# rotationalio/honu

Measured on AMD Instinct MI355X. Metric: GiB/s + records/s device-resident encode+decode, 1M Large(~300KB) object batch, higher is better.
Workload: dtype u8

## Files before the change

honu_amd/csrc/api.hip:

```cpp
#include <stdio.h>
#include <stdlib.h>
#include <string.h>

#include "kernels.h"

using namespace honu;

struct honu_ctx {
    int device;
    uint64_t max_n;
    LaunchGeom geom;
    void *ws;
    uint64_t *counts;
    uint64_t *offs;
    uint64_t *totals;
    DecodeScratch *scratch;
    uint32_t *reg_inline;
    EncAclPos *enc_acl;
    FusedState dec;
    uint64_t lb_bytes;
    ScanState scan;
    uint32_t spec_off;
    int speculate;
    hipStream_t aux;
// ... 24 lines not shown
    return HONU_E_HIP;
}
#define HIPCHK(x)                                  \
    do {                                           \
        hipError_t e_ = (x);                       \
        if (e_ != hipSuccess) return hip_fail(e_, #x); \
    } while (0)

static int32_t arg_fail(const char *what) {
    snprintf(g_last_error, sizeof g_last_error, "invalid argument: %s", what);
    return HONU_E_ARG;
}

static bool aligned(const void *p, uintptr_t a) { return ((uintptr_t)p & (a - 1)) == 0; }

#define FUSED_DECODE_MIN_RECORDS (48ull << 10)

static int fused_blocks(const LaunchGeom &g) {
    const int resident = 2 * g.num_cu;
    return g.lane_blocks > 0 && g.lane_blocks < resident ? g.lane_blocks : resident;
}

template <class T>
static uint64_t carve(T *&p, void *base, uint64_t at, uint64_t count) {
    p = (T *)((uintptr_t)base + at);
    return at + count * sizeof(T);
}

static uint64_t ctx_carve(honu_ctx *c, void *base) {
    const uint64_t n = c->max_n;
    const uint64_t tiles = (n + HONU_WAVE - 1) / HONU_WAVE;
    const uint64_t groups = (tiles / HONU_WAVE + 1) > LB_GROUPS ? tiles / HONU_WAVE + 1 : LB_GROUPS;
    uint64_t at = 0;
    at = carve(c->counts, base, at, 3 * n);
    at = carve(c->offs, base, at, 3 * n);
    at = carve(c->totals, base, at, 4);
    at = carve(c->scratch, base, at, n);
    at = carve(c->reg_inline, base, at, 8 * n);
    at = carve(c->enc_acl, base, at, n);
    at = carve(c->dec.lb, base, at, 1);
    at = carve(c->scan.lb, base, at, 1);
    at = carve(c->dec.status, base, at, 3 * tiles);
    at = carve(c->dec.gstatus, base, at, 3 * groups);
    c->dec.words = 3 * tiles + 3 * groups;
    c->scan.words = scan_status_words(n);
    at = carve(c->scan.status, base, at, c->scan.words);
    return carve(c->geom.copy_tickets, base, at, (uint64_t)COPY_TICKET_LINES * COPY_TICKET_STRIDE);
}

static bool stream_is_restricted(hipStream_t s, int num_cu) {
    int prio = 0;
    if (hipStreamGetPriority(s, &prio) == hipSuccess && prio != 0) return true;
    uint32_t mask[32] = {0};
    const uint32_t words = (uint32_t)((num_cu + 31) / 32);
    if (words > 32 || hipExtStreamGetCUMask(s, words, mask) != hipSuccess) return false;
    bool any = false, all = true;
    for (int i = 0; i < num_cu; i++) {
        const bool on = mask[i / 32] >> (i % 32) & 1u;
        any |= on;
        all &= on;
    }
    return any && !all;
}

static int env_int(const char *name, int dflt) {
#ifdef HONU_AB
    const char *v = getenv(name);
    return v && *v ? atoi(v) : dflt;
#else
    (void)name;
    return dflt;
#endif
}

extern "C" {

uint32_t honu_abi_version(void) { return HONU_ABI_VERSION; }
uint64_t honu_sizeof_meta(void) { return sizeof(honu_meta); }
uint64_t honu_sizeof_acl(void) { return sizeof(honu_acl); }
uint64_t honu_sizeof_collection(void) { return sizeof(honu_collection); }
uint64_t honu_sizeof_index(void) { return sizeof(honu_index); }
uint64_t honu_sizeof_record_info(void) { return sizeof(honu_record_info); }
uint64_t honu_sizeof_seek(void) { return sizeof(honu_seek); }
uint64_t honu_sizeof_list_row(void) { return sizeof(honu_list_row); }
uint64_t honu_sizeof_next(void) { return sizeof(honu_next); }
const char *honu_last_error(void) { return g_last_error; }

const char *honu_status_string(int32_t st) {
    switch (st) {
    case HONU_OK: return "ok";
    case HONU_ERR_BAD_VERSION: return "object is malformed: cannot decode specified version";
    case HONU_ERR_MALFORMED: return "object is malformed: cannot parse data or metadata";
    case HONU_ERR_EOF: return "EOF";
    case HONU_ERR_UNEXPECTED_EOF: return "unexpected EOF";
    case HONU_ERR_NO_LENGTH: return "field not written with length value";
    case HONU_ERR_PARSE_BOOLEAN: return "could not parse boolean value";
    case HONU_ERR_PARSE_VARINT: return "could not parse varint";
    case HONU_ERR_PANIC: return "input on which the Go reference panics";
    case HONU_ERR_CAPACITY: return "output capacity exceeded";
    case HONU_ERR_INPUT: return "input span or list outside its arena";
    case HONU_UNPARSED: return "metadata not decoded (headers only)";
    case HONU_E_ARG: return "invalid argument";
    case HONU_E_WORKSPACE: return "batch larger than the context's reserved records";
    case HONU_E_HIP: return "HIP runtime error";
    case HONU_E_NO_DEVICE: return "no gfx950 device";
    default: return "unknown status";
    }
}

honu_ctx *honu_ctx_create(int device, uint64_t max_records, int32_t *err) {
    int32_t dummy;
    if (!err) err = &dummy;
    *err = HONU_OK;
    int count = 0;
    if (hipGetDeviceCount(&count) != hipSuccess || device < 0 || device >= count) {
        snprintf(g_last_error, sizeof g_last_error, "no HIP device %d (count %d)", device, count);
        *err = HONU_E_NO_DEVICE;
        return nullptr;
    }
    hipDeviceProp_t prop;
    if (hipGetDeviceProperties(&prop, device) != hipSuccess ||
        strncmp(prop.gcnArchName, "gfx950", 6) != 0) {
        snprintf(g_last_error, sizeof g_last_error, "device %d is %s, this build targets gfx950",
                 device, prop.gcnArchName);
        *err = HONU_E_NO_DEVICE;
        return nullptr;
    }
    if (hipSetDevice(device) != hipSuccess) {
        *err = HONU_E_HIP;
        return nullptr;
    }
    honu_ctx *c = (honu_ctx *)calloc(1, sizeof(honu_ctx));
    if (!c) {
        *err = HONU_E_HIP;
        return nullptr;
    }
    auto fail = [&](int32_t e, const char *what) -> honu_ctx * {
        if (what) snprintf(g_last_error, sizeof g_last_error, "%s", what);
        if (c->ev_join) (void)hipEventDestroy(c->ev_join);
        if (c->ev_fork) (void)hipEventDestroy(c->ev_fork);
        if (c->aux) (void)hipStreamDestroy(c->aux);
        if (c->dec.spec_seen) (void)hipHostFree(c->dec.spec_seen);
        if (c->ws) (void)hipFree(c->ws);
        free(c);
        *err = e;
        return nullptr;
    };
    c->device = device;
    c->max_n = max_records ? max_records : 1;
    c->geom.num_cu = prop.multiProcessorCount;
    c->geom.per_record_blocks = env_int("HONU_RECORD_BLOCKS", prop.multiProcessorCount * 8);
    c->geom.lane_blocks = env_int("HONU_LANE_BLOCKS", 0);
    c->geom.copy_blocks = env_int("HONU_COPY_BLOCKS", prop.multiProcessorCount * 2);
    c->geom.record_variant = env_int("HONU_RECORD_VARIANT", 0);
    if (c->geom.record_variant != 5 && c->geom.record_variant != 6)
        c->geom.record_variant = 0;
    c->acl_inplace = env_int("HONU_ACL_INPLACE", 1) != 0;
    c->reg_inplace = env_int("HONU_REGIONS_INPLACE", 1) != 0;
    c->guard_blocks = env_int("HONU_GUARD_BLOCKS", 0);
    if (c->guard_blocks < 0) c->guard_blocks = 0;
    const uint64_t end = ctx_carve(c, nullptr), bytes = end + 256;
    if (hipMalloc(&c->ws, bytes) != hipSuccess) {
        c->ws = nullptr;
        char msg[96];
        snprintf(msg, sizeof msg, "hipMalloc(%llu) failed", (unsigned long long)bytes);
        return fail(HONU_E_HIP, msg);
    }
    if (hipHostMalloc((void **)&c->dec.spec_seen, 2 * sizeof(uint32_t),
                      hipHostMallocMapped | hipHostMallocCoherent) != hipSuccess) {
        c->dec.spec_seen = nullptr;
        return fail(HONU_E_HIP, "hipHostMalloc(spec_seen) failed");
    }
    c->dec.spec_seen[0] = 0;
    c->dec.spec_seen[1] = 0;
    c->speculate = SPECULATE_DEFAULT;
    c->enc_fork = env_int("HONU_ENCODE_FORK", 2);
    if (c->enc_fork < 0 || c->enc_fork > 2) c->enc_fork = 2;
    if (hipStreamCreateWithFlags(&c->aux, hipStreamNonBlocking) != hipSuccess) {
        c->aux = nullptr;
        return fail(HONU_E_HIP, "stream creation failed");
    }
    if (hipEventCreateWithFlags(&c->ev_fork, hipEventDisableTiming) != hipSuccess) {
        c->ev_fork = nullptr;
        return fail(HONU_E_HIP, "event creation failed");
    }
    if (hipEventCreateWithFlags(&c->ev_join, hipEventDisableTiming) != hipSuccess) {
        c->ev_join = nullptr;
        return fail(HONU_E_HIP, "event creation failed");
    }
    ctx_carve(c, c->ws);
    c->lb_bytes = (uint64_t)((uint8_t *)c->ws + end - (uint8_t *)c->dec.lb);
    c->geom.copy_steal = 1;
    c->scan.max_blocks = 4 * prop.multiProcessorCount;
    hipStream_t s = nullptr;
    bool ok = hipStreamCreateWithFlags(&s, hipStreamNonBlocking) == hipSuccess;
    ok = ok && hipMemsetAsync(c->dec.lb, 0, c->lb_bytes, s) == hipSuccess;
    ok = ok && hipStreamSynchronize(s) == hipSuccess;
    if (s) (void)hipStreamDestroy(s);
    if (!ok) return fail(HONU_E_HIP, "look-back state initialisation failed");
    return c;
}

int32_t honu_ctx_reset(honu_ctx *ctx, void *stream) {
    if (!ctx) return arg_fail("ctx");
    HIPCHK(hipSetDevice(ctx->device));
    HIPCHK(hipMemsetAsync(ctx->dec.lb, 0, ctx->lb_bytes, (hipStream_t)stream));
    HIPCHK(hipStreamSynchronize((hipStream_t)stream));
    return HONU_OK;
}

void honu_ctx_destroy(honu_ctx *ctx) {
    if (!ctx) return;
    (void)hipSetDevice(ctx->device);
    (void)hipStreamSynchronize(ctx->aux);
    (void)hipEventDestroy(ctx->ev_fork);
    (void)hipEventDestroy(ctx->ev_join);
    (void)hipStreamDestroy(ctx->aux);
    (void)hipFree(ctx->ws);
    (void)hipHostFree(ctx->dec.spec_seen);
    free(ctx);
}

uint64_t honu_ctx_max_records(const honu_ctx *ctx) { return ctx ? ctx->max_n : 0; }

int32_t honu_ctx_set_param(honu_ctx *ctx, const char *name, int64_t value) {
    if (!ctx || !name) return arg_fail("ctx/name");
    if (!strcmp(name, "copy_blocks") && value > 0) ctx->geom.copy_blocks = (int)value;
    else if (!strcmp(name, "record_blocks") && value > 0) ctx->geom.per_record_blocks = (int)value;
    else if (!strcmp(name, "lane_blocks") && value >= 0) ctx->geom.lane_blocks = (int)value;
    else if (!strcmp(name, "speculate") && value >= 0 && value <= 2) ctx->speculate = (int)value;
    else if (!strcmp(name, "encode_fork") && value >= 0 && value <= 2) ctx->enc_fork = (int)value;
    else if (!strcmp(name, "acl_inplace") && (value == 0 || value == 1)) ctx->acl_inplace = value != 0;
    else if (!strcmp(name, "regions_inplace") && (value == 0 || value == 1)) ctx->reg_inplace = value != 0;
    else if (!strcmp(name, "guard_blocks") && value >= 0 && value <= 65536) ctx->guard_blocks = (int)value;
    else if (!strcmp(name, "speculate_backoff") && value >= 0 && value <= (int64_t)SPEC_BACKOFF_CALLS) {
        __atomic_store_n(ctx->dec.spec_seen, 0u, __ATOMIC_RELAXED);
        ctx->spec_off = (uint32_t)value;
    }
    else if (!strcmp(name, "copy_steal") && (value == 0 || value == 1)) ctx->geom.copy_steal = (int)value;
    else if (!strcmp(name, "copy_variant") || !strcmp(name, "encode_variant") || !strcmp(name, "inline_recovery")) {
        if (value != 0) return arg_fail(name);
    }
    else if (!strcmp(name, "record_variant") &&
             (value == 0 || value == 5 || value == 6))
        ctx->geom.record_variant = (int)value;
    else if (!strcmp(name, "seek_variant") && value >= 0 && value <= 2) ctx->geom.seek_variant = (int)value;
    else return arg_fail(name);
    return HONU_OK;
}

int32_t honu_ctx_get_param(const honu_ctx *ctx, const char *name, int64_t *value) {
    if (!ctx || !name || !value) return arg_fail("ctx/name/value");
    if (!strcmp(name, "copy_blocks")) *value = ctx->geom.copy_blocks;
    else if (!strcmp(name, "record_blocks")) *value = ctx->geom.per_record_blocks;
    else if (!strcmp(name, "lane_blocks")) *value = ctx->geom.lane_blocks;
    else if (!strcmp(name, "speculate")) *value = ctx->speculate;
    else if (!strcmp(name, "encode_fork")) *value = ctx->enc_fork;
    else if (!strcmp(name, "acl_inplace")) *value = ctx->acl_inplace ? 1 : 0;
    else if (!strcmp(name, "regions_inplace")) *value = ctx->reg_inplace ? 1 : 0;
    else if (!strcmp(name, "guard_blocks")) *value = ctx->guard_blocks;
    else if (!strcmp(name, "recoveries"))
        *value = __atomic_load_n(ctx->dec.spec_seen + 1, __ATOMIC_RELAXED);
    else if (!strcmp(name, "speculate_backoff"))
        *value = __atomic_load_n(ctx->dec.spec_seen, __ATOMIC_RELAXED) ? SPEC_BACKOFF_CALLS : ctx->spec_off;
    else if (!strcmp(name, "copy_steal")) *value = ctx->geom.copy_steal;
    else if (!strcmp(name, "copy_variant") || !strcmp(name, "encode_variant") || !strcmp(name, "inline_recovery"))
        *value = 0;
    else if (!strcmp(name, "record_variant")) *value = ctx->geom.record_variant;
    else if (!strcmp(name, "walk_flag_checks")) *value = decode_walk_flag_checks();
    else if (!strcmp(name, "sort_tile")) *value = sort_tile();
    else if (!strcmp(name, "seek_variant")) *value = ctx->geom.seek_variant;
    else if (!strcmp(name, "seek_fence")) *value = seek_fence();
    else if (!strcmp(name, "seek_auto_probes")) *value = (int64_t)seek_auto_probes();
    else if (!strcmp(name, "seek_auto_keys")) *value = (int64_t)seek_auto_keys();
    else if (!strcmp(name, "merge_tile")) *value = merge_tile();
    else if (!strcmp(name, "delete_tile")) *value = delete_tile();
    else if (!strcmp(name, "list_tile")) *value = list_tile();
    else if (!strcmp(name, "list_stage")) *value = list_stage();
    else if (!strcmp(name, "filter_tile")) *value = filter_tile();
    else if (!strcmp(name, "compare_tile")) *value = compare_tile();
    else if (!strcmp(name, "compare_stage")) *value = compare_stage();
    else return arg_fail(name);
    return HONU_OK;
}

int32_t honu_encode_sizes(honu_ctx *ctx, const honu_meta *d_meta, uint64_t var_len,
                          const honu_acl *d_acl, uint64_t acl_len, const uint32_t *d_regions,
                          uint64_t regions_len, const uint64_t *d_payload_off, uint64_t n,
                          uint64_t *d_sizes, int32_t *d_status, void *stream) {
    if (!ctx) return arg_fail("ctx");
    if (n && (!d_meta || !d_payload_off || !d_sizes)) return arg_fail("null pointer");
    if (!aligned(d_meta, 16)) return arg_fail("rows must be 16-byte aligned");
    if (!aligned(d_acl, 4) || !aligned(d_regions, 4)) return arg_fail("tables must be 4-byte aligned");
    HIPCHK(hipSetDevice(ctx->device));
    HIPCHK(launch_encode_sizes_grp(d_meta, var_len, d_acl, acl_len, d_regions, regions_len,
                                   d_payload_off, n, d_sizes, d_status, ctx->geom.lane_blocks,
                                   (hipStream_t)stream));
    return HONU_OK;
}

int32_t honu_exclusive_scan(honu_ctx *ctx, const uint64_t *d_in, uint64_t n, uint64_t *d_out,
                            void *stream) {
    if (!ctx) return arg_fail("ctx");
    if (n > ctx->max_n) return HONU_E_WORKSPACE;
    HIPCHK(hipSetDevice(ctx->device));
    HIPCHK(launch_scan(d_in, n, 1, d_out, d_out + n, ctx->scan, (hipStream_t)stream));
    return HONU_OK;
}

static int32_t encode_records(honu_ctx *ctx, const honu_meta *d_meta, const uint8_t *d_var,
                              const honu_acl *d_acl, const uint32_t *d_regions, const uint8_t *units,
                              const uint64_t *d_payload_off, uint64_t n, uint8_t *d_out,
                              uint64_t out_cap, const uint64_t *d_out_off, int32_t *d_status,
                              void *stream) {
    if (!ctx) return arg_fail("ctx");
    if (n && (!d_meta || !d_payload_off || !d_out || !d_out_off || !d_status))
        return arg_fail("null pointer");
    if (!aligned(d_out, 16) || !aligned(d_meta, 16))
        return arg_fail("records arena and rows must be 16-byte aligned");
    if (!aligned(d_acl, 4) || !aligned(d_regions, 4)) return arg_fail("tables must be 4-byte aligned");
    HIPCHK(hipSetDevice(ctx->device));
    if (n > ctx->max_n) return HONU_E_WORKSPACE;
    ctx->enc_form = units ? 2 : 1;
    hipStream_t s = (hipStream_t)stream;
    const bool fork = ctx->enc_fork == 1 ||
                      (ctx->enc_fork == 2 && ctx->geom.lane_blocks > 0 && n &&
                       !stream_is_restricted(s, ctx->geom.num_cu));
    if (fork && n) {
        HIPCHK(hipEventRecord(ctx->ev_fork, s));
        HIPCHK(hipStreamWaitEvent(ctx->aux, ctx->ev_fork, 0));
        HIPCHK(launch_encode_acl_grp_self(d_meta, d_acl, d_payload_off, n, d_out, out_cap, d_out_off, d_status,
                                          ctx->geom.lane_blocks, ctx->aux));
        HIPCHK(hipEventRecord(ctx->ev_join, ctx->aux));
        HIPCHK(launch_encode_meta_lane(d_meta, d_var, d_acl, d_regions, d_payload_off, n, d_out,
                                       out_cap, d_out_off, d_status, ctx->enc_acl,
                                       ctx->geom.lane_blocks, ctx->geom.num_cu, units, s));
        HIPCHK(hipStreamWaitEvent(s, ctx->ev_join, 0));
        return HONU_OK;
    }
    HIPCHK(launch_encode_meta_lane(d_meta, d_var, d_acl, d_regions, d_payload_off, n, d_out,
                                   out_cap, d_out_off, d_status, ctx->enc_acl,
                                   ctx->geom.lane_blocks, ctx->geom.num_cu, units, s));
    HIPCHK(launch_encode_acl_grp(d_meta, d_acl, n, d_out, d_status, ctx->enc_acl,
                                 ctx->geom.lane_blocks, s));
    return HONU_OK;
}

int32_t honu_encode_records(honu_ctx *ctx, const honu_meta *d_meta, const uint8_t *d_var,
                            const honu_acl *d_acl, const uint32_t *d_regions,
                            const uint64_t *d_payload_off, uint64_t n, uint8_t *d_out,
                            uint64_t out_cap, const uint64_t *d_out_off, int32_t *d_status,
                            void *stream) {
    return encode_records(ctx, d_meta, d_var, d_acl, d_regions, nullptr, d_payload_off, n, d_out, out_cap,
                          d_out_off, d_status, stream);
}

int32_t honu_encode_records_units(honu_ctx *ctx, const honu_meta *d_meta, const uint8_t *d_var,
                                  const honu_acl *d_acl, const uint32_t *d_regions,
                                  const uint8_t *d_payload, const uint64_t *d_payload_off, uint64_t n,
                                  uint8_t *d_out, uint64_t out_cap, const uint64_t *d_out_off,
                                  int32_t *d_status, void *stream) {
    if (n && !d_payload) return arg_fail("null pointer");
    return encode_records(ctx, d_meta, d_var, d_acl, d_regions, d_payload, d_payload_off, n, d_out, out_cap,
                          d_out_off, d_status, stream);
}

static int32_t encode_payloads(honu_ctx *ctx, const uint8_t *d_payload, const uint64_t *d_payload_off,
                               uint64_t n, uint8_t *d_out, uint64_t out_cap, const uint64_t *d_out_off,
                               const int32_t *d_status, bool units, void *stream) {
    if (!ctx) return arg_fail("ctx");
    if (n && (!d_payload_off || !d_out || !d_out_off || !d_status)) return arg_fail("null pointer");
    if (!aligned(d_out, 16)) return arg_fail("records arena must be 16-byte aligned");
    if (ctx->enc_form && ctx->enc_form != (units ? 2 : 1))
        return arg_fail(units ? "honu_encode_payloads_units after honu_encode_records (mixed forms)"
                              : "honu_encode_payloads after honu_encode_records_units (mixed forms)");
    HIPCHK(hipSetDevice(ctx->device));
    HIPCHK(launch_encode_copy(copy_geom(ctx), d_payload, d_payload_off, n, d_out, out_cap, d_out_off,
                              d_status, units, (hipStream_t)stream));
    return HONU_OK;
}

int32_t honu_encode_payloads(honu_ctx *ctx, const uint8_t *d_payload, const uint64_t *d_payload_off,
                             uint64_t n, uint8_t *d_out, uint64_t out_cap, const uint64_t *d_out_off,
                             const int32_t *d_status, void *stream) {
    return encode_payloads(ctx, d_payload, d_payload_off, n, d_out, out_cap, d_out_off, d_status, false, stream);
}

int32_t honu_encode_payloads_units(honu_ctx *ctx, const uint8_t *d_payload, const uint64_t *d_payload_off,
                                   uint64_t n, uint8_t *d_out, uint64_t out_cap, const uint64_t *d_out_off,
                                   const int32_t *d_status, void *stream) {
    return encode_payloads(ctx, d_payload, d_payload_off, n, d_out, out_cap, d_out_off, d_status, true, stream);
}

int32_t honu_encode(honu_ctx *ctx, const honu_meta *d_meta, const uint8_t *d_var, uint64_t var_len,
                    const honu_acl *d_acl, uint64_t acl_len, const uint32_t *d_regions,
                    uint64_t regions_len, const uint8_t *d_payload, const uint64_t *d_payload_off,
                    uint64_t n, uint8_t *d_out, uint64_t out_cap, const uint64_t *d_out_off,
                    int32_t *d_status, void *stream) {
    (void)var_len;
    (void)acl_len;
    (void)regions_len;
    if (!d_payload) {
        int32_t st = honu_encode_records(ctx, d_meta, d_var, d_acl, d_regions, d_payload_off, n, d_out,
                                         out_cap, d_out_off, d_status, stream);
        if (st) return st;
        return honu_encode_payloads(ctx, d_payload, d_payload_off, n, d_out, out_cap, d_out_off, d_status,
                                    stream);
    }
    int32_t st = honu_encode_records_units(ctx, d_meta, d_var, d_acl, d_regions, d_payload, d_payload_off, n,
                                           d_out, out_cap, d_out_off, d_status, stream);
    if (st) return st;
    return honu_encode_payloads_units(ctx, d_payload, d_payload_off, n, d_out, out_cap, d_out_off,
                                      d_status, stream);
}

int32_t honu_marshal_batch(honu_ctx *ctx, const honu_meta *d_meta, const uint8_t *d_var,
                           uint64_t var_len, const honu_acl *d_acl, uint64_t acl_len,
                           const uint32_t *d_regions, uint64_t regions_len,
                           const uint8_t *d_payload, const uint64_t *d_payload_off, uint64_t n,
                           uint8_t *d_out, uint64_t out_cap, uint64_t *d_out_off,
                           int32_t *d_status, void *stream) {
    if (!ctx) return arg_fail("ctx");
    if (n > ctx->max_n) return HONU_E_WORKSPACE;
    if (n && (!d_meta || !d_payload_off || !d_out || !d_out_off || !d_status)) return arg_fail("null pointer");
    if (!aligned(d_out, 16) || !aligned(d_meta, 16))
        return arg_fail("records arena and rows must be 16-byte aligned");
    int32_t st = honu_encode_sizes(ctx, d_meta, var_len, d_acl, acl_len, d_regions, regions_len,
                                   d_payload_off, n, d_out_off, d_status, stream);
    if (st) return st;
    st = honu_exclusive_scan(ctx, d_out_off, n, d_out_off, stream);
    if (st) return st;
    return honu_encode(ctx, d_meta, d_var, var_len, d_acl, acl_len, d_regions, regions_len,
                       d_payload, d_payload_off, n, d_out, out_cap, d_out_off, d_status, stream);
}

int32_t honu_decode_parse(honu_ctx *ctx, const uint8_t *d_rec, const uint64_t *d_rec_off,
                          uint64_t n, honu_meta *d_meta, honu_record_info *d_info, void *stream) {
    if (!ctx) return arg_fail("ctx");
    if (n > ctx->max_n) return HONU_E_WORKSPACE;
    if (n && (!d_rec || !d_rec_off || !d_meta || !d_info)) return arg_fail("null pointer");
    if (!aligned(d_rec, 16) || !aligned(d_meta, 16) || !aligned(d_info, 8))
        return arg_fail("records arena and rows must be 16-byte aligned");
    HIPCHK(hipSetDevice(ctx->device));
    HIPCHK(launch_decode_parse_win(d_rec, d_rec_off, n, d_meta, d_info, ctx->scratch,
                                   ctx->reg_inline, ctx->counts, ctx->geom.lane_blocks,
                                   ctx->acl_inplace, ctx->reg_inplace, (hipStream_t)stream));
    return HONU_OK;
}

int32_t honu_decode_tables(honu_ctx *ctx, const uint8_t *d_rec, uint64_t n, honu_meta *d_meta,
                           honu_record_info *d_info, honu_acl *d_acl, uint64_t acl_cap,
                           uint32_t *d_regions, uint64_t regions_cap, uint8_t *d_data,
                           uint64_t data_cap, uint64_t *d_totals, void *stream) {
    if (!ctx) return arg_fail("ctx");
    if (n > ctx->max_n) return HONU_E_WORKSPACE;
    if (!aligned(d_acl, 4) || !aligned(d_regions, 4) || !aligned(d_data, 16))
        return arg_fail("tables 4-byte / data arena 16-byte aligned");
    if (acl_cap && !d_acl) return arg_fail("acl table");
    if (regions_cap && !d_regions) return arg_fail("region table");
    HIPCHK(hipSetDevice(ctx->device));
    hipStream_t s = (hipStream_t)stream;
    uint64_t *tot = d_totals ? d_totals : ctx->totals;
    HIPCHK(launch_scan(ctx->counts, n, 3, ctx->offs, tot, ctx->scan, s));
    HIPCHK(launch_decode_fill_grp(d_rec, n, d_meta, d_info, ctx->scratch, ctx->reg_inline,
                                  ctx->counts, ctx->offs, d_acl, acl_cap, d_regions, regions_cap,
                                  d_data, data_cap, ctx->geom.lane_blocks, s));
    return HONU_OK;
}

int32_t honu_decode_payloads(honu_ctx *ctx, const uint8_t *d_rec, uint64_t n,
                             const honu_record_info *d_info, uint8_t *d_data,
                             const uint64_t *d_totals, void *stream) {
    if (!ctx) return arg_fail("ctx");
    if (n > ctx->max_n) return HONU_E_WORKSPACE;
    if (!d_data || !aligned(d_data, 16)) return arg_fail("data arena");
    HIPCHK(hipSetDevice(ctx->device));
    const uint64_t *tot = d_totals ? d_totals : ctx->totals;
    HIPCHK(launch_decode_copy(copy_geom(ctx), d_rec, n, d_info, ctx->scratch, ctx->offs, tot, d_data,
                              (hipStream_t)stream));
    return HONU_OK;
}

int32_t honu_decode_fill(honu_ctx *ctx, const uint8_t *d_rec, const uint64_t *d_rec_off,
                         uint64_t n, honu_meta *d_meta, honu_record_info *d_info,
                         honu_acl *d_acl, uint64_t acl_cap, uint32_t *d_regions,
                         uint64_t regions_cap, uint8_t *d_data, uint64_t data_cap,
                         uint64_t *d_totals, void *stream) {
    (void)d_rec_off;
    int32_t st = honu_decode_tables(ctx, d_rec, n, d_meta, d_info, d_acl, acl_cap, d_regions,
                                    regions_cap, d_data, data_cap, d_totals, stream);
    if (st || !d_data) return st;
    return honu_decode_payloads(ctx, d_rec, n, d_info, d_data, d_totals, stream);
}

int32_t honu_decode_records(honu_ctx *ctx, const uint8_t *d_rec, const uint64_t *d_rec_off,
// ... 530 lines not shown
```

honu_amd/csrc/kernels.h:

```cpp
#pragma once

#include "common.h"
#include "lookback.h"

namespace honu {

struct DecodeScratch {
    uint64_t acl_pos;
    uint64_t regions_pos;
    uint64_t data_src;
    uint64_t rec_end;
};

#define GRP_ACL_FAST (1ull << 63)
#define GRP_REG_INLINE (1ull << 62)
#define GRP_ACL_A0_SHIFT 56
#define GRP_ACL_A0(pos) (((pos) >> GRP_ACL_A0_SHIFT) & 15ull)
#define GRP_ACL_TL_SHIFT 53
#define GRP_ACL_TL(pos) (((pos) >> GRP_ACL_TL_SHIFT) & 7ull)
#define GRP_POS_MASK ((1ull << GRP_ACL_TL_SHIFT) - 1)
#define ACL_ALL_PRESENT (1ull << 63)
#define PAYLOAD_UNIT 64ull

HONU_DEV void acl_enc_words(const honu_acl *e, uint32_t d[5]) {
    const uint32_t *w = reinterpret_cast<const uint32_t *>(e);
    const uint32_t e0 = w[0], e1 = w[1], e2 = w[2], e3 = w[3], e4 = w[4];
    d[0] = 1u | (e0 << 8);
    d[1] = (e0 >> 24) | (e1 << 8);
    d[2] = (e1 >> 24) | (e2 << 8);
    d[3] = (e2 >> 24) | (e3 << 8);
    d[4] = (e3 >> 24) | ((e4 & 0xFF) << 8);
}

HONU_DEV u32x4 acl_chunk(const honu_acl *A, uint64_t na, uint64_t P, uint64_t X) {
    const uint64_t j0 = (X - P) / 18;
    uint32_t b[10];
    acl_enc_words(A + j0, b);
    b[5] = b[6] = b[7] = b[8] = b[9] = 0;
    if (j0 + 1 < na) {
        uint32_t d[5];
        acl_enc_words(A + j0 + 1, d);
        b[4] = (b[4] & 0xFFFF) | (d[0] << 16);
        b[5] = (d[0] >> 16) | (d[1] << 16);
        b[6] = (d[1] >> 16) | (d[2] << 16);
        b[7] = (d[2] >> 16) | (d[3] << 16);
        b[8] = (d[3] >> 16) | (d[4] << 16);
    }
    const uint32_t off = (uint32_t)(X - (P + 18 * j0));
    const uint32_t q = off >> 2, sh = off & 3;
    uint32_t o[4];
#pragma unroll
    for (int k = 0; k < 4; k++) {
        uint32_t w0 = b[k], w1 = b[k + 1];
#pragma unroll
        for (int t = 1; t <= 4; t++)
            if ((uint32_t)t == q) {
                w0 = b[t + k];
                w1 = b[t + k + 1];
            }
        o[k] = __builtin_amdgcn_alignbyte(w1, w0, sh);
    }
    return u32x4{o[0], o[1], o[2], o[3]};
}

struct LaunchGeom {
    int num_cu;
    int per_record_blocks;
    int lane_blocks;
    int copy_blocks;
    int record_variant;
    int seek_variant;
    uint32_t *copy_tickets;
    int copy_steal;
};
#define COPY_TICKET_STRIDE 32u
#define COPY_TICKET_LINES 64u

hipError_t launch_encode_copy(const LaunchGeom &g, const uint8_t *payload,
                              const uint64_t *payload_off, uint64_t n, uint8_t *out,
                              uint64_t out_cap, const uint64_t *out_off, const int32_t *status,
                              bool units, hipStream_t s);

hipError_t launch_decode_copy(const LaunchGeom &g, const uint8_t *rec, uint64_t n,
                              const honu_record_info *info, const DecodeScratch *scratch,
                              const uint64_t *offs, const uint64_t *totals, uint8_t *data,
                              hipStream_t s);
hipError_t launch_decode_keys(const LaunchGeom &g, const honu_meta *meta,
                              const honu_record_info *info, uint64_t n, uint8_t *keys,
                              int32_t *key_status, hipStream_t s);

struct EncAclPos {
    uint64_t pos;
    uint64_t acl_off;
    uint64_t acl_count;
    uint64_t carried;
};
#define ENC_ACL_SIZED (1ull << 63)

hipError_t launch_encode_meta_lane(const honu_meta *meta, const uint8_t *var, const honu_acl *acl,
                                   const uint32_t *reg, const uint64_t *payload_off, uint64_t n,
                                   uint8_t *out, uint64_t out_cap, const uint64_t *out_off,
                                   int32_t *status, EncAclPos *acl_out, int max_blocks, int num_cu,
                                   const uint8_t *payload, hipStream_t s);
hipError_t launch_encode_acl_grp(const honu_meta *meta, const honu_acl *acl, uint64_t n,
                                 uint8_t *out, int32_t *status, const EncAclPos *acl_pos,
                                 int max_blocks, hipStream_t s);
hipError_t launch_encode_acl_grp_self(const honu_meta *meta, const honu_acl *acl, const uint64_t *payload_off,
                                      uint64_t n, uint8_t *out, uint64_t out_cap, const uint64_t *out_off,
                                      int32_t *status, int max_blocks, hipStream_t s);

hipError_t launch_encode_sizes_grp(const honu_meta *meta, uint64_t var_len, const honu_acl *acl,
                                   uint64_t acl_len, const uint32_t *reg, uint64_t reg_len,
                                   const uint64_t *payload_off, uint64_t n, uint64_t *sizes,
                                   int32_t *status, int max_blocks, hipStream_t s);
hipError_t launch_decode_fill_grp(const uint8_t *rec, uint64_t n, honu_meta *meta,
                                  honu_record_info *info, const DecodeScratch *scratch,
                                  const uint32_t *reg_inline, const uint64_t *counts,
                                  const uint64_t *offs, honu_acl *acl, uint64_t acl_cap,
                                  uint32_t *reg, uint64_t reg_cap, uint8_t *data,
                                  uint64_t data_cap, int max_blocks, hipStream_t s);

int decode_walk_flag_checks();
struct DecodeOut {
    honu_meta *meta;
    honu_record_info *info;
    honu_acl *acl;
    uint64_t acl_cap;
    uint32_t *reg;
    uint64_t reg_cap;
    uint64_t data_cap;
    int materialize;
    DecodeScratch *scratch;
    uint64_t *offs;
    uint64_t *totals;
    bool reg_inplace;
};
struct FusedState {
    LbState *lb;
    uint64_t *status, *gstatus;
    uint64_t words;
    uint32_t *spec_seen;
};
struct FusedOpts {
    int max_blocks;
    int guard_blocks;
    bool speculate;
    bool acl_inplace;
};
hipError_t launch_decode_fused(const uint8_t *rec, const uint64_t *rec_off, uint64_t n,
                               const DecodeOut &O, const FusedState &F, const FusedOpts &opt, hipStream_t s);

hipError_t launch_decode_parse_win(const uint8_t *rec, const uint64_t *rec_off, uint64_t n,
                                   honu_meta *meta, honu_record_info *info,
                                   DecodeScratch *scratch, uint32_t *reg_inline, uint64_t *counts,
                                   int max_blocks, bool inplace, bool reg_inplace, hipStream_t s);

hipError_t launch_system_sizes(const honu_collection *rows, uint64_t var_len, const honu_acl *acl,
                               uint64_t acl_len, const uint32_t *reg, uint64_t reg_len,
                               const honu_index *idx, uint64_t idx_len, uint64_t n,
                               uint64_t *sizes, int32_t *status, hipStream_t s);
hipError_t launch_system_encode(const honu_collection *rows, const uint8_t *var,
                                const honu_acl *acl, const uint32_t *reg, const honu_index *idx,
                                uint64_t n, uint8_t *out, uint64_t out_cap,
                                const uint64_t *out_off, int32_t *status, hipStream_t s);
hipError_t launch_system_parse(const uint8_t *rec, const uint64_t *rec_off, uint64_t n,
                               bool headless, honu_collection *rows, int32_t *status,
                               DecodeScratch *scratch, uint64_t *counts, hipStream_t s);
hipError_t launch_system_fill(const uint8_t *rec, uint64_t n, honu_collection *rows,
                              int32_t *status, const DecodeScratch *scratch,
                              const uint64_t *counts, const uint64_t *offs, honu_acl *acl,
                              uint64_t acl_cap, uint32_t *reg, uint64_t reg_cap, honu_index *idx,
                              uint64_t idx_cap, hipStream_t s);

hipError_t launch_decode_headers(const uint8_t *rec, const uint64_t *rec_off, uint64_t n,
                                 honu_record_info *info, hipStream_t s);
hipError_t launch_decode_spans(const uint8_t *rec, const uint64_t *rec_off, uint64_t n,
                               honu_record_info *info, DecodeScratch *scratch, uint64_t *counts,
                               hipStream_t s);
hipError_t launch_decode_data_place(uint64_t n, honu_record_info *info, const uint64_t *offs,
                                    uint64_t data_cap, hipStream_t s);
hipError_t launch_span_copy(const LaunchGeom &g, const uint8_t *rec, uint64_t n,
                            const honu_record_info *info, const DecodeScratch *scratch,
                            const uint64_t *offs, uint8_t *data, hipStream_t s);

struct ScanState {
    LbState *lb;
    uint64_t *status;
    uint64_t words;
    int max_blocks;
};
uint64_t scan_status_words(uint64_t n);
hipError_t launch_scan(const uint64_t *in, uint64_t n, int K, uint64_t *out, uint64_t *totals,
                       const ScanState &S, hipStream_t s);

inline uint64_t up256(uint64_t x) { return (x + 255) & ~255ull; }

struct SortWork {
    uint32_t *plan;
    u32x4 *key[2];
    uint32_t *idx[2];
    uint64_t *col;
    uint64_t *table;
};
uint32_t sort_tile();
uint64_t sort_workspace_bytes(uint64_t n);
SortWork sort_carve(void *work, uint64_t n);
hipError_t launch_sort_keys(const uint8_t *keys, const int32_t *status, uint64_t n, uint32_t *order,
                            uint8_t *sorted, uint64_t *valid, void *work, const ScanState &S,
                            uint64_t scan_rows, hipStream_t s);
hipError_t launch_key_objects(const uint8_t *keys, const uint32_t *order, const uint64_t *valid, uint64_t n,
                              uint64_t *obj_off, uint32_t *latest, uint64_t *objects, void *work,
                              const ScanState &S, hipStream_t s);

uint32_t seek_fence();
uint64_t seek_auto_probes();
uint64_t seek_auto_keys();
hipError_t launch_key_seek(int variant, int num_cu, const uint8_t *sorted, const uint64_t *valid, uint64_t n,
                           const uint8_t *probes, const int32_t *pstatus, uint32_t probe_len, uint64_t m,
                           const uint32_t *order, const honu_record_info *info, honu_seek *out, hipStream_t s);

uint32_t merge_tile();
hipError_t launch_key_merge(const uint8_t *sa, const uint32_t *oa, const uint64_t *valid_a, uint64_t na,
                            const uint8_t *sb, const uint32_t *ob, const uint64_t *valid_b, uint64_t nb,
                            uint32_t b_base, uint8_t *out, uint32_t *order, uint64_t *valid_out, hipStream_t s);

uint32_t delete_tile();
uint64_t delete_tiles(uint64_t n);
uint64_t delete_workspace_bytes(uint64_t n);
hipError_t launch_key_delete(const uint8_t *sorted, const uint32_t *order, const uint64_t *valid, uint64_t n,
                             const uint8_t *del, const uint64_t *valid_del, uint64_t m, uint32_t probe_len,
                             uint32_t flags, uint8_t *out, uint32_t *order_out, uint64_t *valid_out,
                             uint64_t *removed, void *work, const ScanState &S, hipStream_t s);

uint32_t list_tile();
uint32_t list_stage();
hipError_t launch_key_list(int num_cu, const uint8_t *sorted, const uint32_t *order, const uint64_t *valid, uint64_t n,
                           const honu_seek *ranges, uint64_t m, uint32_t limit, uint32_t flags,
                           const uint64_t *obj_off, const uint64_t *objects, const honu_record_info *info,
                           uint64_t *range_off, honu_list_row *rows, uint8_t *keys_out, uint64_t cap,
                           uint64_t *total, const ScanState &S, hipStream_t s);

hipError_t launch_key_fetch(const LaunchGeom &g, const honu_list_row *rows, const uint64_t *total, uint64_t cap,
                            const uint8_t *rec, const uint64_t *rec_off, uint64_t nrec, uint64_t rec_bytes,
                            uint32_t flags, uint64_t *val_off, int32_t *status, uint8_t *values, uint64_t val_cap,
                            uint64_t *val_total, const ScanState &S, hipStream_t s);
hipError_t launch_fetch_copy(const LaunchGeom &g, const honu_list_row *rows, uint64_t n, const uint8_t *rec,
                             const uint64_t *rec_off, const uint64_t *val_off, uint8_t *values,
                             uint64_t val_cap, hipStream_t s);

uint32_t filter_tile();
uint64_t filter_tiles(uint64_t cap);
uint64_t filter_workspace_bytes(uint64_t cap);
hipError_t launch_key_filter(const honu_list_row *rows, const uint8_t *keys, const uint64_t *range_off, uint64_t m,
                             const uint64_t *total, uint64_t cap, uint32_t flags, const uint64_t *valid, uint64_t n,
                             const uint64_t *obj_off, const uint32_t *latest, const uint64_t *objects,
                             const honu_record_info *info, honu_list_row *rows_out, uint8_t *keys_out,
// ... 33 lines not shown
```

honu_amd/csrc/lane.hip:

```cpp
#include "kernels.h"
#include "lane.h"

namespace honu {

#define OFF(f) ((int)offsetof(honu_meta, f))

template <int RING> constexpr uint32_t enc_wave_bytes() { return (RING > 0 ? RING : 1) * HONU_WAVE * 16; }

template <bool SKIP_ACL, int RING>
HONU_DEV void k_encode_meta_lane_one(uint64_t i, const honu_meta &m, const uint8_t *__restrict__ var,
    const honu_acl *__restrict__ acl, const uint32_t *__restrict__ reg,
    const uint64_t *__restrict__ payload_off, uint8_t *__restrict__ out,
    uint64_t out_cap, const uint64_t *__restrict__ out_off, int32_t *__restrict__ status,
    EncAclPos *__restrict__ acl_out, u32x4 *ring, const uint8_t *__restrict__ payload) {
    if (status[i] != HONU_OK) return;
    const uint64_t beg = out_off[i], end = out_off[i + 1];
    if (end > out_cap) {
        status[i] = HONU_ERR_CAPACITY;
        return;
    }
    const uint64_t dlen = payload_off[i + 1] - payload_off[i];
    const uint64_t pos = encode_record_lane<SKIP_ACL, SKIP_ACL ? RING : 0>(
        m, var, acl, reg, dlen, beg, end, out, ring, payload ? payload + payload_off[i] : nullptr);
    if constexpr (SKIP_ACL)
        acl_out[i] = EncAclPos{pos, m.acl_off, m.acl_count,
                               m.acl_bytes | ((m.present & HONU_ACL_SIZED) ? ENC_ACL_SIZED : 0)};
}

HONU_DEV void load_row(const honu_meta *__restrict__ src, honu_meta &m) {
    const u32x4 *s = reinterpret_cast<const u32x4 *>(src);
    u32x4 *d = reinterpret_cast<u32x4 *>(&m);
#pragma unroll
    for (int k = 0; k < 22; k++) d[k] = s[k];
}

template <bool SKIP_ACL, int RING, bool UNITS = false>
__global__ __launch_bounds__(HONU_BLOCK) void k_encode_meta_lane(
    const honu_meta *__restrict__ meta, const uint8_t *__restrict__ var,
    const honu_acl *__restrict__ acl, const uint32_t *__restrict__ reg,
    const uint64_t *__restrict__ payload_off, uint64_t n, uint8_t *__restrict__ out,
    uint64_t out_cap, const uint64_t *__restrict__ out_off, int32_t *__restrict__ status,
    EncAclPos *__restrict__ acl_out, const uint8_t *__restrict__ payload) {
    constexpr uint32_t WAVE_BYTES = enc_wave_bytes<RING>();
    __shared__ __attribute__((aligned(16))) uint8_t smem[HONU_WAVES_PER_BLOCK * WAVE_BYTES];
    uint8_t *area = smem + (threadIdx.x / HONU_WAVE) * WAVE_BYTES;
    u32x4 *ring = reinterpret_cast<u32x4 *>(area) + lane_id();
    for (uint64_t t0 = (uint64_t)blockIdx.x * HONU_BLOCK + (threadIdx.x & ~(uint64_t)(HONU_WAVE - 1)); t0 < n;
         t0 += (uint64_t)gridDim.x * HONU_BLOCK) {
        const uint64_t i = t0 + lane_id();
        ESTAMP(0);
        honu_meta m;
        if (i < n) {
            load_row(meta + i, m);
            k_encode_meta_lane_one<SKIP_ACL, RING>(i, m, var, acl, reg, payload_off, out, out_cap, out_off, status,
                                             acl_out, ring, UNITS ? payload : nullptr);
        }
    }
}

#undef OFF

template <bool SPANS>
__global__ __launch_bounds__(HONU_BLOCK) void k_decode_headers(
    const uint8_t *__restrict__ rec, const uint64_t *__restrict__ rec_off, uint64_t n,
    honu_record_info *__restrict__ info, DecodeScratch *__restrict__ scratch,
    uint64_t *__restrict__ counts) {
    for (uint64_t i = (uint64_t)blockIdx.x * HONU_BLOCK + threadIdx.x; i < n;
         i += (uint64_t)gridDim.x * HONU_BLOCK) {
        const uint64_t beg = rec_off[i], end = rec_off[i + 1];
        const uint64_t len = end - beg;
        uint32_t ver = 0;
        int64_t d = -1, b = -1;
        if (len) {
            uint64_t lo, hi;
            lane_fetch16(rec, beg, end, lo, hi);
            ver = (uint32_t)(lo & 0xFF);
            if (len >= 3) {
                const uint32_t wl = (uint32_t)(len - 2 < 10 ? len - 2 : 10);
                uint64_t x;
                const uint32_t k = uvarint_window((lo >> 8) | (hi << 56), hi >> 8, wl, x);
                if (k) {
                    d = (int64_t)x;
                    b = k;
                }
            }
        }
        const bool v1 = ver == HONU_STORAGE_VERSION;
        honu_record_info inf;
        inf.data_off = 0;
        inf.data_len = 0;
        if (!v1) inf.data_status = HONU_ERR_BAD_VERSION;
        else if (d < 0) inf.data_status = HONU_ERR_MALFORMED;
        else if (d == 0) inf.data_status = HONU_OK;
        else if ((uint64_t)d > len - 1 - (uint64_t)b) inf.data_status = HONU_ERR_PANIC;
        else {
            inf.data_status = HONU_OK;
            inf.data_off = beg + 1 + (uint64_t)b;
            inf.data_len = (uint64_t)d;
        }
        inf.meta_status = HONU_UNPARSED;
        inf.storage_version = (uint8_t)ver;
        inf.tombstone = (v1 && d == 0) ? 1 : 0;
#pragma unroll
        for (int k = 0; k < 6; k++) inf._pad[k] = 0;
        if constexpr (SPANS) {
            scratch[i].data_src = inf.data_off;
            counts[i] = (inf.data_len + 15) & ~15ull;
        }
        store_info(info + i, inf);
    }
}

__global__ __launch_bounds__(HONU_BLOCK) void k_decode_data_place(
    uint64_t n, honu_record_info *__restrict__ info, const uint64_t *__restrict__ offs,
    uint64_t data_cap) {
    for (uint64_t i = (uint64_t)blockIdx.x * HONU_BLOCK + threadIdx.x; i < n;
         i += (uint64_t)gridDim.x * HONU_BLOCK) {
        honu_record_info *p = info + i;
        if (p->data_status != HONU_OK || !p->data_len) continue;
        const uint64_t o = offs[i];
        if (o > data_cap || p->data_len > data_cap - o) {
            p->data_status = HONU_ERR_CAPACITY;
            p->data_off = 0;
            p->data_len = 0;
        } else {
            p->data_off = o;
        }
    }
}

static dim3 flat_grid(uint64_t n) {
    const uint64_t b = (n + HONU_BLOCK - 1) / HONU_BLOCK;
    return dim3((unsigned)(b > 65536 ? 65536 : b));
}

hipError_t launch_decode_headers(const uint8_t *rec, const uint64_t *rec_off, uint64_t n,
                                 honu_record_info *info, hipStream_t s) {
    if (n == 0) return hipSuccess;
    hipLaunchKernelGGL(k_decode_headers<false>, flat_grid(n), dim3(HONU_BLOCK), 0, s, rec, rec_off,
                       n, info, nullptr, nullptr);
    return hipGetLastError();
}

hipError_t launch_decode_spans(const uint8_t *rec, const uint64_t *rec_off, uint64_t n,
                               honu_record_info *info, DecodeScratch *scratch, uint64_t *counts,
                               hipStream_t s) {
    if (n == 0) return hipSuccess;
    hipLaunchKernelGGL(k_decode_headers<true>, flat_grid(n), dim3(HONU_BLOCK), 0, s, rec, rec_off, n,
                       info, scratch, counts);
    return hipGetLastError();
}

hipError_t launch_decode_data_place(uint64_t n, honu_record_info *info, const uint64_t *offs,
                                    uint64_t data_cap, hipStream_t s) {
    if (n == 0) return hipSuccess;
    hipLaunchKernelGGL(k_decode_data_place, flat_grid(n), dim3(HONU_BLOCK), 0, s, n, info, offs,
                       data_cap);
    return hipGetLastError();
}

static dim3 lane_grid(uint64_t n, int cap) {
    const uint64_t b = (n + HONU_BLOCK - 1) / HONU_BLOCK;
    return dim3((unsigned)(cap > 0 && b > (uint64_t)cap ? (uint64_t)cap : b));
}

hipError_t launch_encode_meta_lane(const honu_meta *meta, const uint8_t *var, const honu_acl *acl,
                                   const uint32_t *reg, const uint64_t *payload_off, uint64_t n,
                                   uint8_t *out, uint64_t out_cap, const uint64_t *out_off,
                                   int32_t *status, EncAclPos *acl_out, int max_blocks, int num_cu,
                                   const uint8_t *payload, hipStream_t s) {
    if (n == 0) return hipSuccess;
    if (!acl_out) return hipErrorInvalidValue;
    const dim3 grid = lane_grid(n, max_blocks);
#ifdef ENC_LINE_MIN_TILES_N
    const uint64_t line_min_tiles = ENC_LINE_MIN_TILES_N;
    (void)num_cu;
#else
    const uint64_t resident_blocks = grid.x < 2u * (uint64_t)num_cu ? grid.x : 2u * (uint64_t)num_cu;
    const uint64_t line_min_tiles = HONU_WAVES_PER_BLOCK * resident_blocks;
#endif
    const bool line = (n + HONU_WAVE - 1) / HONU_WAVE > line_min_tiles;
#define HONU_META_LANE(RG, U)                                                                        \
    hipLaunchKernelGGL((k_encode_meta_lane<true, RG, U>), grid, dim3(HONU_BLOCK), 0, s, meta, var, acl, \
                       reg, payload_off, n, out, out_cap, out_off, status, acl_out, payload)
    if (line && payload) HONU_META_LANE(16, true);
    else if (line) HONU_META_LANE(16, false);
    else if (payload) HONU_META_LANE(8, true);
    else HONU_META_LANE(8, false);
#undef HONU_META_LANE
    return hipGetLastError();
}

}

#ifdef HONU_ENC_TIMING
extern "C" int32_t honu_debug_enc_stamps(void *host, uint64_t waves) {
    if (waves > (1 << 16)) waves = 1 << 16;
    return hipMemcpyFromSymbol(host, HIP_SYMBOL(honu::g_enc_stamps),
                               waves * ENC_STAMPS * sizeof(uint64_t)) == hipSuccess ? 0 : -3;
}
#endif
```

Measured before the change: 1378.

## Stage encoder meta rows through LDS with coalesced wave loads for line path

Each wave now loads its tile of 352-byte meta rows with coalesced 16-byte loads spread across lanes, stages them through shared memory in two halves, and each lane then reads its own row from LDS. Previously every lane read its own row directly with strided loads. The per-record status and offsets are loaded up front as well. By default the staged path is used for the large-batch 'line' variant, and the direct path is kept for ring-8. This adds LDS footprint and wave syncs in exchange for better global memory coalescing.

```diff
diff --git a/honu_amd/csrc/api.hip b/honu_amd/csrc/api.hip
--- a/honu_amd/csrc/api.hip
+++ b/honu_amd/csrc/api.hip
@@ -200,6 +200,7 @@
     c->geom.per_record_blocks = env_int("HONU_RECORD_BLOCKS", prop.multiProcessorCount * 8);
     c->geom.lane_blocks = env_int("HONU_LANE_BLOCKS", 0);
     c->geom.copy_blocks = env_int("HONU_COPY_BLOCKS", prop.multiProcessorCount * 2);
+    c->geom.enc_row_direct = env_int("HONU_ENC_ROW_DIRECT", -1);
     c->geom.record_variant = env_int("HONU_RECORD_VARIANT", 0);
     if (c->geom.record_variant != 5 && c->geom.record_variant != 6)
         c->geom.record_variant = 0;
@@ -382,13 +383,15 @@
         HIPCHK(hipEventRecord(ctx->ev_join, ctx->aux));
         HIPCHK(launch_encode_meta_lane(d_meta, d_var, d_acl, d_regions, d_payload_off, n, d_out,
                                        out_cap, d_out_off, d_status, ctx->enc_acl,
-                                       ctx->geom.lane_blocks, ctx->geom.num_cu, units, s));
+                                       ctx->geom.lane_blocks, ctx->geom.num_cu,
+                                       ctx->geom.enc_row_direct, units, s));
         HIPCHK(hipStreamWaitEvent(s, ctx->ev_join, 0));
         return HONU_OK;
     }
     HIPCHK(launch_encode_meta_lane(d_meta, d_var, d_acl, d_regions, d_payload_off, n, d_out,
                                    out_cap, d_out_off, d_status, ctx->enc_acl,
-                                   ctx->geom.lane_blocks, ctx->geom.num_cu, units, s));
+                                   ctx->geom.lane_blocks, ctx->geom.num_cu,
+                                   ctx->geom.enc_row_direct, units, s));
     HIPCHK(launch_encode_acl_grp(d_meta, d_acl, n, d_out, d_status, ctx->enc_acl,
                                  ctx->geom.lane_blocks, s));
     return HONU_OK;
diff --git a/honu_amd/csrc/kernels.h b/honu_amd/csrc/kernels.h
--- a/honu_amd/csrc/kernels.h
+++ b/honu_amd/csrc/kernels.h
@@ -72,6 +72,7 @@
     int seek_variant;
     uint32_t *copy_tickets;
     int copy_steal;
+    int enc_row_direct;
 };
 #define COPY_TICKET_STRIDE 32u
 #define COPY_TICKET_LINES 64u
@@ -101,7 +102,7 @@
                                    const uint32_t *reg, const uint64_t *payload_off, uint64_t n,
                                    uint8_t *out, uint64_t out_cap, const uint64_t *out_off,
                                    int32_t *status, EncAclPos *acl_out, int max_blocks, int num_cu,
-                                   const uint8_t *payload, hipStream_t s);
+                                   int row_direct, const uint8_t *payload, hipStream_t s);
 hipError_t launch_encode_acl_grp(const honu_meta *meta, const honu_acl *acl, uint64_t n,
                                  uint8_t *out, int32_t *status, const EncAclPos *acl_pos,
                                  int max_blocks, hipStream_t s);
diff --git a/honu_amd/csrc/lane.hip b/honu_amd/csrc/lane.hip
--- a/honu_amd/csrc/lane.hip
+++ b/honu_amd/csrc/lane.hip
@@ -5,23 +5,42 @@
 
 #define OFF(f) ((int)offsetof(honu_meta, f))
 
-template <int RING> constexpr uint32_t enc_wave_bytes() { return (RING > 0 ? RING : 1) * HONU_WAVE * 16; }
+constexpr uint32_t ROW_CHUNKS = sizeof(honu_meta) / 16;
+constexpr uint32_t ENC_STAGE_ROWS = HONU_WAVE / 2;
+constexpr uint32_t ENC_STAGE_BYTES = ENC_STAGE_ROWS * sizeof(honu_meta);
+static_assert(sizeof(honu_meta) % 16 == 0 && ROW_CHUNKS % 2 == 0,
+              "a half tile is a whole number of 64-chunk loads (ROW_CHUNKS / 2 per lane)");
+template <int RING, bool DIRECT> constexpr uint32_t enc_wave_bytes() {
+    constexpr uint32_t ring = (RING > 0 ? RING : 1) * HONU_WAVE * 16;
+    return DIRECT || ring > ENC_STAGE_BYTES ? ring : ENC_STAGE_BYTES;
+}
+static_assert(2 * HONU_WAVES_PER_BLOCK * enc_wave_bytes<16, false>() <= 160 * 1024 &&
+              2 * HONU_WAVES_PER_BLOCK * enc_wave_bytes<8, false>() <= 160 * 1024 &&
+              enc_wave_bytes<8, false>() >= ENC_STAGE_BYTES && enc_wave_bytes<16, false>() >= ENC_STAGE_BYTES,
+              "two workgroups of the lane encoder per CU, each wave's area holding half a tile's rows");
+
+struct EncRecIn {
+    int32_t status;
+    uint64_t beg, end, dlen;
+};
+HONU_DEV EncRecIn load_rec_in(uint64_t i, const uint64_t *__restrict__ payload_off,
+                              const uint64_t *__restrict__ out_off, const int32_t *__restrict__ status) {
+    return EncRecIn{status[i], out_off[i], out_off[i + 1], payload_off[i + 1] - payload_off[i]};
+}
 
 template <bool SKIP_ACL, int RING>
-HONU_DEV void k_encode_meta_lane_one(uint64_t i, const honu_meta &m, const uint8_t *__restrict__ var,
-    const honu_acl *__restrict__ acl, const uint32_t *__restrict__ reg,
+HONU_DEV void k_encode_meta_lane_one(uint64_t i, const honu_meta &m, const EncRecIn &in,
+    const uint8_t *__restrict__ var, const honu_acl *__restrict__ acl, const uint32_t *__restrict__ reg,
     const uint64_t *__restrict__ payload_off, uint8_t *__restrict__ out,
-    uint64_t out_cap, const uint64_t *__restrict__ out_off, int32_t *__restrict__ status,
+    uint64_t out_cap, int32_t *__restrict__ status,
     EncAclPos *__restrict__ acl_out, u32x4 *ring, const uint8_t *__restrict__ payload) {
-    if (status[i] != HONU_OK) return;
-    const uint64_t beg = out_off[i], end = out_off[i + 1];
-    if (end > out_cap) {
+    if (in.status != HONU_OK) return;
+    if (in.end > out_cap) {
         status[i] = HONU_ERR_CAPACITY;
         return;
     }
-    const uint64_t dlen = payload_off[i + 1] - payload_off[i];
     const uint64_t pos = encode_record_lane<SKIP_ACL, SKIP_ACL ? RING : 0>(
-        m, var, acl, reg, dlen, beg, end, out, ring, payload ? payload + payload_off[i] : nullptr);
+        m, var, acl, reg, in.dlen, in.beg, in.end, out, ring, payload ? payload + payload_off[i] : nullptr);
     if constexpr (SKIP_ACL)
         acl_out[i] = EncAclPos{pos, m.acl_off, m.acl_count,
                                m.acl_bytes | ((m.present & HONU_ACL_SIZED) ? ENC_ACL_SIZED : 0)};
@@ -31,17 +50,44 @@
     const u32x4 *s = reinterpret_cast<const u32x4 *>(src);
     u32x4 *d = reinterpret_cast<u32x4 *>(&m);
 #pragma unroll
-    for (int k = 0; k < 22; k++) d[k] = s[k];
-}
-
-template <bool SKIP_ACL, int RING, bool UNITS = false>
+    for (int k = 0; k < (int)ROW_CHUNKS; k++) d[k] = s[k];
+}
+
+HONU_DEV void load_rows_staged(const honu_meta *__restrict__ tile, uint32_t rows, u32x4 *area, honu_meta &m) {
+    constexpr int H = ROW_CHUNKS / 2;
+    const uint32_t lane = lane_id();
+    const u32x4 *s = reinterpret_cast<const u32x4 *>(tile);
+    const uint32_t last = rows * ROW_CHUNKS - 1;
+    u32x4 v[2 * H];
+#pragma unroll
+    for (int k = 0; k < 2 * H; k++) {
+        const uint32_t c = k * HONU_WAVE + lane;
+        v[k] = s[c < last ? c : last];
+    }
+    u32x4 *d = reinterpret_cast<u32x4 *>(&m);
+    const u32x4 *row = area + (lane & (ENC_STAGE_ROWS - 1)) * ROW_CHUNKS;
+#pragma unroll
+    for (int h = 0; h < 2; h++) {
+        wave_sync();
+#pragma unroll
+        for (int k = 0; k < H; k++) area[k * HONU_WAVE + lane] = v[h * H + k];
+        wave_sync();
+        if ((lane / ENC_STAGE_ROWS) == (uint32_t)h) {
+#pragma unroll
+            for (int k = 0; k < (int)ROW_CHUNKS; k++) d[k] = row[k];
+        }
+    }
+    wave_sync();
+}
+
+template <bool SKIP_ACL, int RING, bool UNITS, bool DIRECT>
 __global__ __launch_bounds__(HONU_BLOCK) void k_encode_meta_lane(
     const honu_meta *__restrict__ meta, const uint8_t *__restrict__ var,
     const honu_acl *__restrict__ acl, const uint32_t *__restrict__ reg,
     const uint64_t *__restrict__ payload_off, uint64_t n, uint8_t *__restrict__ out,
     uint64_t out_cap, const uint64_t *__restrict__ out_off, int32_t *__restrict__ status,
     EncAclPos *__restrict__ acl_out, const uint8_t *__restrict__ payload) {
-    constexpr uint32_t WAVE_BYTES = enc_wave_bytes<RING>();
+    constexpr uint32_t WAVE_BYTES = enc_wave_bytes<RING, DIRECT>();
     __shared__ __attribute__((aligned(16))) uint8_t smem[HONU_WAVES_PER_BLOCK * WAVE_BYTES];
     uint8_t *area = smem + (threadIdx.x / HONU_WAVE) * WAVE_BYTES;
     u32x4 *ring = reinterpret_cast<u32x4 *>(area) + lane_id();
@@ -50,11 +96,20 @@
         const uint64_t i = t0 + lane_id();
         ESTAMP(0);
         honu_meta m;
-        if (i < n) {
-            load_row(meta + i, m);
-            k_encode_meta_lane_one<SKIP_ACL, RING>(i, m, var, acl, reg, payload_off, out, out_cap, out_off, status,
-                                             acl_out, ring, UNITS ? payload : nullptr);
-        }
+        EncRecIn in{HONU_ERR_INPUT, 0, 0, 0};
+        if constexpr (DIRECT) {
+            if (i < n) {
+                load_row(meta + i, m);
+                in = load_rec_in(i, payload_off, out_off, status);
+            }
+        } else {
+            in = load_rec_in(i < n ? i : n - 1, payload_off, out_off, status);
+            load_rows_staged(meta + t0, (uint32_t)(n - t0 < HONU_WAVE ? n - t0 : HONU_WAVE),
+                             reinterpret_cast<u32x4 *>(area), m);
+        }
+        if (i < n)
+            k_encode_meta_lane_one<SKIP_ACL, RING>(i, m, in, var, acl, reg, payload_off, out, out_cap, status,
+                                                   acl_out, ring, UNITS ? payload : nullptr);
     }
 }
 
@@ -168,7 +223,7 @@
                                    const uint32_t *reg, const uint64_t *payload_off, uint64_t n,
                                    uint8_t *out, uint64_t out_cap, const uint64_t *out_off,
                                    int32_t *status, EncAclPos *acl_out, int max_blocks, int num_cu,
-                                   const uint8_t *payload, hipStream_t s) {
+                                   int row_direct, const uint8_t *payload, hipStream_t s) {
     if (n == 0) return hipSuccess;
     if (!acl_out) return hipErrorInvalidValue;
     const dim3 grid = lane_grid(n, max_blocks);
@@ -180,13 +235,28 @@
     const uint64_t line_min_tiles = HONU_WAVES_PER_BLOCK * resident_blocks;
 #endif
     const bool line = (n + HONU_WAVE - 1) / HONU_WAVE > line_min_tiles;
-#define HONU_META_LANE(RG, U)                                                                        \
-    hipLaunchKernelGGL((k_encode_meta_lane<true, RG, U>), grid, dim3(HONU_BLOCK), 0, s, meta, var, acl, \
+#define HONU_META_LANE(RG, U, D)                                                                        \
+    hipLaunchKernelGGL((k_encode_meta_lane<true, RG, U, D>), grid, dim3(HONU_BLOCK), 0, s, meta, var, acl, \
                        reg, payload_off, n, out, out_cap, out_off, status, acl_out, payload)
-    if (line && payload) HONU_META_LANE(16, true);
-    else if (line) HONU_META_LANE(16, false);
-    else if (payload) HONU_META_LANE(8, true);
-    else HONU_META_LANE(8, false);
+#ifdef HONU_AB
+    const bool line_direct = row_direct > 0, ring8_direct = row_direct != 0;
+    if (line && line_direct) {
+        if (payload) HONU_META_LANE(16, true, true);
+        else HONU_META_LANE(16, false, true);
+        return hipGetLastError();
+    }
+    if (!line && !ring8_direct) {
+        if (payload) HONU_META_LANE(8, true, false);
+        else HONU_META_LANE(8, false, false);
+        return hipGetLastError();
+    }
+#else
+    (void)row_direct;
+#endif
+    if (line && payload) HONU_META_LANE(16, true, false);
+    else if (line) HONU_META_LANE(16, false, false);
+    else if (payload) HONU_META_LANE(8, true, true);
+    else HONU_META_LANE(8, false, true);
 #undef HONU_META_LANE
     return hipGetLastError();
 }
```

Result: no change. 1376, median of 3 (-0.2%).
